# Baran-phys/IEA-GAN

Measured on AMD Instinct MI355X. Metric: events/sec (40x250x768) per G+D train step, higher is better.
Workload: dtype bf16; 1 GPU; BASELINE configs[1]: 1 event (40x1x256x768) per GPU per step, hinge loss only, RRM on, DiffAugment on, ortho reg + Adam + EMA in the timed region, fp32 master weights, 4 synthetic events in rotation; parallelism=dp1, hip_graph=True

## Files before the change

iea-gan_amd/_hip.py:

```python
from __future__ import annotations

import ctypes as C
import os

import torch

_HERE = os.path.dirname(os.path.abspath(__file__))
LIB_PATH = os.path.join(_HERE, "libieagan_hip.so")
CONV_FP8_NOSCALE = 8
CONV_FP8 = 4
CONV_FORCE_WS64 = 32
CONV_NO_WS64 = 16
CONV_NO_LDS_WEIGHTS = 2
CONV_FORCE_GATHER = 1
B1_TP32 = 4
BWD_NO_REDUCE = 16
PXD_BINS = 251
PXD_CLUSTER_COLUMNS = {"size_spectrum": (0, 64), "charge_spectrum": (64, 256), "seed_spectrum": (320, 256), "size_u_spectrum": (576, 32),
                       "size_v_spectrum": (608, 32)}
PXD_CLUSTER_BINS = 640
PXD_MAP_U, PXD_MAP_V = 25, 48
PXD_MATCH_COUNTERS = ("hits", "matched", "changed", "shared", "lost")
PXD_MATCH_COLUMNS = {"residual_u": (5, 64), "residual_v": (69, 64), "purity": (133, 32)}
PXD_MATCH_BINS = 165
PXD_CORR_MAX_COLUMNS, PXD_CORR_MAX_EVENTS = 1024, 65535
PROLOGUE_BWD_SLOTS = 64
AUG_SLOTS = 128
BNB_REPL = 8
STAT_REPL = 32
SN_FIELDS = 16

vp, fp, lp, ip = C.c_void_p, C.c_void_p, C.c_void_p, C.c_void_p


class SrcDesc(C.Structure):
    _fields_ = [("x", vp), ("Cx", C.c_int), ("Hs", C.c_int), ("Ws", C.c_int), ("rs", C.c_int),
                ("scale", vp), ("shift", vp), ("aff_nstride", C.c_int), ("relu", C.c_int)]


class ConvDesc(C.Structure):
    _fields_ = [("N", C.c_int), ("H", C.c_int), ("W", C.c_int), ("Cin", C.c_int), ("Cout", C.c_int),
                ("taps", C.c_int), ("Kpad", C.c_int), ("src", SrcDesc), ("w", vp), ("bias", vp),
                ("ra", vp), ("Cra", C.c_int), ("Ca", C.c_int), ("ra_rs", C.c_int), ("ra_scale", C.c_float), ("rb", vp),
                ("Crb", C.c_int), ("mask", vp), ("out", vp), ("stats", vp), ("n_per_event", C.c_int), ("flags", C.c_int),
                ("bnb_scale", vp), ("bnb_shift", vp), ("bnb_nstride", C.c_int), ("bnb_relu", C.c_int), ("stats_slots", C.c_int)]


class WgradDesc(C.Structure):
    _fields_ = [("N", C.c_int), ("H", C.c_int), ("W", C.c_int), ("Cin", C.c_int), ("Cout", C.c_int),
                ("taps", C.c_int), ("Kpad", C.c_int), ("src", SrcDesc), ("g", vp), ("Cg", C.c_int),
                ("dw", vp), ("tiles_per_block", C.c_int), ("pad_rows", C.c_int), ("partials", vp), ("colsum", vp)]


class Conv1x1BwdDesc(C.Structure):
    _fields_ = [("N", C.c_int), ("H", C.c_int), ("W", C.c_int), ("Cin", C.c_int), ("Cout", C.c_int), ("Kpad", C.c_int),
                ("Kpad2", C.c_int), ("src", SrcDesc), ("g", vp), ("Cg", C.c_int), ("y", vp), ("dstat", vp), ("n_per_event", C.c_int),
                ("geff_out", vp), ("w_bwd", vp), ("lg", vp), ("lC", C.c_int), ("lCa", C.c_int), ("lmode", C.c_int), ("dx", vp),
                ("out_mode", C.c_int), ("bn_acc", vp), ("dw", vp), ("partials", vp), ("colsum", vp), ("flags", C.c_int), ("bn_slots", C.c_int)]


class Conv3x3BwdDesc(C.Structure):
    _fields_ = [("N", C.c_int), ("H", C.c_int), ("W", C.c_int), ("C", C.c_int), ("Kpad", C.c_int), ("src", SrcDesc), ("g", vp), ("Cg", C.c_int),
                ("y", vp), ("dstat", vp), ("n_per_event", C.c_int), ("w_bwd", vp), ("dx", vp), ("bn_acc", vp), ("dw", vp), ("partials", vp),
                ("colsum", vp), ("flags", C.c_int), ("bn_slots", C.c_int)]


class ReduceItem(C.Structure):
    _fields_ = [("partials", vp), ("dw", vp), ("S", C.c_int), ("Cout", C.c_int), ("Kpad", C.c_int), ("K", C.c_int)]


class DStemDesc(C.Structure):
    _fields_ = [("img", vp), ("N", C.c_int), ("H", C.c_int), ("W", C.c_int), ("w_in", vp), ("b_in", vp), ("w1", vp), ("b1", vp), ("wsc", vp),
                ("bsc", vp), ("h1", vp), ("p0", vp), ("sc", vp), ("dh1", vp), ("dp0", vp), ("w1_bwd", vp), ("dw_in", vp), ("db_in", vp),
                ("dw1", vp), ("db1", vp)]


class ProfRec(C.Structure):
    _fields_ = [("name", C.c_char * 96), ("launches", C.c_long), ("ms", C.c_double),
                ("flops", C.c_double), ("bytes", C.c_double), ("bytes_min", C.c_double)]


ABI_VERSION = 12
i, f, l = C.c_int, C.c_float, C.c_long
_SIGS = {
    "ieagan_abi_version": [],
    "ieagan_prof_enable": [i],
    "ieagan_prof_reset": [],
    "ieagan_prof_collect": [C.POINTER(ProfRec), i],
    "ieagan_conv_forward": [C.POINTER(ConvDesc), vp],
    "ieagan_conv_wgrad": [C.POINTER(WgradDesc), i, vp],
    "ieagan_conv_wgrad_workspace": [C.POINTER(WgradDesc), i],
    "ieagan_conv1x1_bwd": [C.POINTER(Conv1x1BwdDesc), vp],
    "ieagan_conv1x1_bwd_workspace": [C.POINTER(Conv1x1BwdDesc)],
    "ieagan_conv1x1_bwd_supported": [i, i, i, i],
    "ieagan_conv3x3_bwd": [C.POINTER(Conv3x3BwdDesc), vp],
# ... 147 lines not shown
```

iea-gan_amd/csrc/conv3x3_ws.hip:

```cpp
#include "common.h"
#include "conv_args.h"
#include "conv3x3_tile.h"

#define WS_H 8
#define WS_W 32

template <bool AFF, bool RELU, int RS, int CIN, bool BNB, bool MPF, int NCW, bool FULL>
__global__ __launch_bounds__((NCW + 4) * 64, (NCW == 4 ? 4 : 3)) void conv3x3_ws_kernel(ConvArgs a, int tiles_w, int tiles_h, int tpe, int tpb, int nblk, int bpe) {
    constexpr int NT = CIN / 16;
    constexpr int AW = WS_W + 2, AH = WS_H + 2;
    constexpr int PS = CIN * 2 + 16;
    constexpr int KP = ((9 * CIN + 31) / 32) * 32;
    constexpr int WSB = KP * 2 + 16;
    constexpr int CH = CIN / 8;
    constexpr int TOT = AH * AW * CH;
    constexpr int PF = (TOT + 255) / 256;
    constexpr int HALO_BYTES = AH * AW * PS;
    extern __shared__ __attribute__((aligned(16))) char smem_all[];
    constexpr int RPW = WS_H / NCW, MTW = 2 * RPW;
    __shared__ float red[NCW * NT * 16 * 2];
    __shared__ __attribute__((aligned(32))) float aff_all[4 * 64];
    char* wlds = smem_all;
    char* halo0 = smem_all + NT * 16 * WSB;
    float* epi_all = (float*)(halo0 + 2 * HALO_BYTES);

    const int lane = threadIdx.x & 63, wave = threadIdx.x >> 6;
    const bool consumer = wave < NCW;
    const int lr = lane & 15, lg = lane >> 4;
    const int H = a.H, W = a.W;
    const TileRun run = tile_run(nblk, 1, bpe, tpe, tpb);
    const int t0 = run.t0, ntl = run.t1 - run.t0;

    for (int idx = threadIdx.x; idx < NT * 16 * (KP / 8); idx += (NCW + 4) * 64) {
        const int row = idx / (KP / 8), kc = idx - row * (KP / 8);
        *(bf16x8*)(wlds + row * WSB + kc * 16) = *(const bf16x8*)((const bf16*)a.w + (long)row * KP + kc * 8);
    }

    auto tile_coords = [&](int t, int& n, int& h0, int& w0) { tile_origin<WS_H, WS_W>(t, tiles_w, tiles_h, n, h0, w0); };

    if (!consumer) {
        const int ptid = threadIdx.x - NCW * 64;
        bf16x8 rawA[PF], rawB[PF];
        unsigned okA = 0, okB = 0;
        float* aff_w = aff_all + (wave & 3) * 64;
        int aff_n = -1;
        auto load_tile = [&](int t, bf16x8(&raw)[PF], unsigned& okmask) {
            int n, h0, w0;
            tile_coords(t, n, h0, w0);
            halo_request<RS, CH, AW, TOT, 256>(a.src, H, W, n, h0, w0, ptid, raw, okmask);
        };
        auto store_tile = [&](int t, const bf16x8(&raw)[PF], unsigned okmask, char* dst) {
            int n, h0, w0;
            tile_coords(t, n, h0, w0);
            if (AFF && n != aff_n) {
                wave_fence();
                const int c = lane & 31;
                if (c < CIN) aff_w[lane] = (lane < 32 ? a.src.scale : a.src.shift)[(long)n * a.src.aff_nstride + c];
                wave_fence();
                aff_n = n;
            }
#pragma unroll
            for (int j = 0; j < PF; ++j) {
                const int idx = ptid + j * 256;
                if (idx >= TOT) continue;
                const int hp = idx / CH, cc = idx - hp * CH;
                *(bf16x8*)(dst + hp * PS + cc * 16) = prologue_chunk<AFF, RELU>(raw[j], okmask & (1u << j), aff_w + cc * 8, aff_w + 32 + cc * 8);
            }
        };
        auto produce = [&](int r, bf16x8(&raw)[PF], unsigned& okmask) {
            if (r + 1 < ntl) store_tile(t0 + r + 1, raw, okmask, halo0 + ((r + 1) & 1) * HALO_BYTES);
            load_tile(t0 + min(r + 3, ntl - 1), raw, okmask);
        };
        if (ntl <= 0) {
            __syncthreads();
            return;
        }
        load_tile(t0, rawA, okA);
        store_tile(t0, rawA, okA, halo0);
        load_tile(t0 + min(1, ntl - 1), rawB, okB);
        load_tile(t0 + min(2, ntl - 1), rawA, okA);
        __syncthreads();
        for (int r = 0; r < ntl; r += 2) {
            produce(r, rawB, okB);
            __syncthreads();
            if (r + 1 >= ntl) break;
            produce(r + 1, rawA, okA);
            __syncthreads();
        }
        if (a.stats != nullptr) __syncthreads();
        return;
    }

    float s1[8], s2[8];
#pragma unroll
    for (int i = 0; i < 8; ++i) s1[i] = s2[i] = 0.f;
    int pbase[MTW];
#pragma unroll
    for (int mt = 0; mt < MTW; ++mt) pbase[mt] = ((RPW * wave + (mt >> 1)) * AW + (mt & 1) * 16 + lr) * PS;
    float* epi = epi_all + wave * EpiLds<NT>::FLOATS;
    constexpr int CPP = NT * 2, EIT = (32 * CPP) / 64;
    const int ecc = lane % CPP;
    float bias_r[8];
    load_bias8<NT>(a, 0, bias_r);
    constexpr bool has_mask = MPF;
    bf16x8 mk_cur[RPW * EIT], mk_nxt[RPW * EIT];
    auto mask_request = [&](int t, bf16x8(&mk)[RPW * EIT]) {
        int n, h0, w0;
        tile_coords(t, n, h0, w0);
#pragma unroll
        for (int half = 0; half < RPW; ++half)
#pragma unroll
            for (int it = 0; it < EIT; ++it) {
                const int hh = h0 + RPW * wave + half, ww = w0 + (it * 64 + lane) / CPP;
                if (FULL) {
                    mk[half * EIT + it] = *(const bf16x8*)((const bf16*)a.mask + (((long)n * H + hh) * W + ww) * CIN + ecc * 8);
                } else {
                    mk[half * EIT + it] = zero8();
                    if (hh < H && ww < W) mk[half * EIT + it] = *(const bf16x8*)((const bf16*)a.mask + (((long)n * H + hh) * W + ww) * CIN + ecc * 8);
                }
            }
    };
    if (has_mask && ntl > 0) mask_request(t0, mk_cur);
    __syncthreads();
    for (int r = 0; r < ntl; ++r) {
        const char* smem = halo0 + (r & 1) * HALO_BYTES;
        int n, h0, w0;
        tile_coords(t0 + r, n, h0, w0);
        f32x4 acc[MTW][NT];
#pragma unroll
        for (int mt = 0; mt < MTW; ++mt)
#pragma unroll
            for (int nt = 0; nt < NT; ++nt) acc[mt][nt] = (f32x4){0.f, 0.f, 0.f, 0.f};
        constexpr int KS = KP / 32;
        bf16x8 bq[CIN >= 32 ? 2 : 1][NT], aq[CIN >= 32 ? 2 : 1][MTW];
        auto ldb = [&](int ks, bf16x8(&b)[NT]) {
#pragma unroll
            for (int nt = 0; nt < NT; ++nt) b[nt] = *(const bf16x8*)(wlds + (nt * 16 + lr) * WSB + (ks * 32 + lg * 8) * 2);
        };
        auto lda = [&](int ks, bf16x8(&x)[MTW]) {
            const int k = ks * 32 + lg * 8;
            int tap = k / CIN;
            const int c = k - tap * CIN;
            const bool kval = tap < 9;
            if (!kval) tap = 0;
            const int toff = ((tap / 3) * AW + (tap - (tap / 3) * 3)) * PS + c * 2;
#pragma unroll
            for (int mt = 0; mt < MTW; ++mt) {
                x[mt] = *(const bf16x8*)(smem + pbase[mt] + toff);
                if (!kval) x[mt] = zero8();
            }
        };
        if constexpr (CIN >= 32) {
            ldb(0, bq[0]);
            lda(0, aq[0]);
#pragma unroll
            for (int ks = 0; ks < KS; ++ks) {
                if (ks + 1 < KS) {
                    ldb(ks + 1, bq[(ks + 1) & 1]);
                    lda(ks + 1, aq[(ks + 1) & 1]);
                }
                __builtin_amdgcn_sched_barrier(0);
#pragma unroll
                for (int mt = 0; mt < MTW; ++mt)
#pragma unroll
                    for (int nt = 0; nt < NT; ++nt)
                        acc[mt][nt] = __builtin_amdgcn_mfma_f32_16x16x32_bf16(aq[ks & 1][mt], bq[ks & 1][nt], acc[mt][nt], 0, 0, 0);
                __builtin_amdgcn_sched_barrier(0);
            }
        } else {
#pragma unroll
            for (int ks = 0; ks < KS; ++ks) {
                ldb(ks, bq[0]);
                lda(ks, aq[0]);
#pragma unroll
                for (int mt = 0; mt < MTW; ++mt)
#pragma unroll
                    for (int nt = 0; nt < NT; ++nt)
                        acc[mt][nt] = __builtin_amdgcn_mfma_f32_16x16x32_bf16(aq[0][mt], bq[0][nt], acc[mt][nt], 0, 0, 0);
            }
        }
#pragma unroll
        for (int half = 0; half < RPW; ++half) {
            const tile_pix<2, FULL> pix(n, h0, w0, 2 * (RPW * wave + half), H, W);
            const f32x4(&sub)[2][NT] = *reinterpret_cast<const f32x4(*)[2][NT]>(&acc[2 * half]);
            if (half == 0 && has_mask) mask_request(t0 + min(r + 1, ntl - 1), mk_nxt);
            if (has_mask) conv_epilogue<BNB, NT>(a, sub, epi, 0, pix, s1, s2, bias_r, &mk_cur[half * EIT]);
            else conv_epilogue<BNB, NT>(a, sub, epi, 0, pix, s1, s2, bias_r, nullptr);
        }
        if (has_mask) {
#pragma unroll
            for (int i = 0; i < RPW * EIT; ++i) mk_cur[i] = mk_nxt[i];
        }
        __syncthreads();
    }
    if (a.stats != nullptr && ntl > 0) stats_flush<NT, NCW>(a, s1, s2, 0, red, epi_all, run.bid, run.event);
}

template <bool AFF, bool RELU, int RS, bool BNB, bool MPF, bool FULL>
static int ws_launch_f(const ConvArgs& a, hipStream_t st) {
    const TilePlan p = tile_plan_events(a, WS_H, WS_W, a.Cin == 16 ? 512 : 256, 1);
#define WS_GO(CINV, NCWV)                                                                                                    \
    {                                                                                                                        \
        constexpr int NTV = CINV / 16;                                                                                       \
        constexpr int KPV = ((9 * CINV + 31) / 32) * 32;                                                                     \
        size_t tail = (size_t)NCWV * EpiLds<NTV>::FLOATS * 4;                                                                \
        if (tail < (size_t)NCWV * STATS_SX_FLOATS * 4) tail = (size_t)NCWV * STATS_SX_FLOATS * 4;                             \
        const size_t lds = (size_t)NTV * 16 * (KPV * 2 + 16) + 2 * (size_t)(WS_H + 2) * (WS_W + 2) * (CINV * 2 + 16) + tail;  \
        CONV_PLAN_POINT(p.bpe, 1)                                                                                            \
        constexpr auto kern = conv3x3_ws_kernel<AFF, RELU, RS, CINV, BNB, MPF, NCWV, FULL>;                                  \
        if (reserve_lds<kern>(lds, "conv3x3_ws") != 0) return IEAGAN_ELAUNCH;                                                \
        hipLaunchKernelGGL(kern, dim3(p.nblk), dim3((NCWV + 4) * 64), lds, st, a, p.tiles_w, p.tiles_h, p.tpe, p.tpb, p.nblk, p.bpe); \
    }
    WS_GO(16, 4)
#undef WS_GO
    return 1;
}

template <bool AFF, bool RELU, int RS, bool BNB, bool MPF>
static int ws_launch_c(const ConvArgs& a, hipStream_t st) {
    if (a.H % WS_H == 0 && a.W % WS_W == 0) return ws_launch_f<AFF, RELU, RS, BNB, MPF, true>(a, st);
    return ws_launch_f<AFF, RELU, RS, BNB, MPF, false>(a, st);
}

int conv3x3_ws_launch(const ConvArgs& a, hipStream_t st) {
    if (a.taps != 9 || a.Cin != a.Cout || a.Cin != 16 || a.src.rs == 2) return 0;
    if (a.Kpad != ((9 * a.Cin + 31) / 32) * 32 || a.src.Cx % 8 != 0) return 0;
    const int tiles = a.N * ((a.W + WS_W - 1) / WS_W) * ((a.H + WS_H - 1) / WS_H);
    if (tiles < 1024) return 0;
    const bool aff = a.src.scale != nullptr, relu = a.src.relu != 0;
    if (aff && !relu) return 0;
    if (a.mask != nullptr) {
        if (aff || relu || a.src.rs != 0) return 0;
        return a.bnb_scale != nullptr ? ws_launch_c<false, false, 0, true, true>(a, st) : ws_launch_c<false, false, 0, false, true>(a, st);
    }
    return dispatch_prologue(a, [&](auto AFF, auto RELU, auto RS, auto BNB) {
        if constexpr (BNB() || (AFF() && !RELU())) return 0;
        else return ws_launch_c<AFF(), RELU(), RS(), false, false>(a, st);
    });
}
```

iea-gan_amd/csrc/conv_igemm.hip:

```cpp
#include "common.h"
#include "conv_args.h"
#include "conv3x3_tile.h"
#include <stdio.h>

template <int TAPS, bool AFF, bool RELU, int RS, int NT, bool LAFF, bool BNB = false>
__global__ __launch_bounds__(256, 4) void conv_gather_kernel(ConvArgs a) {
    constexpr int EROWS = (NT >= 2) ? 16 : 32;
    __shared__ __attribute__((aligned(16))) float epi[4 * EROWS * EpiLds<NT>::LDW];
    __shared__ float red[4 * NT * 16 * 2];
    __shared__ __attribute__((aligned(32))) float aff_s[LAFF ? 2 * AFF_MAXC : 8];
    const int lane = threadIdx.x & 63, wave = threadIdx.x >> 6;
    const int lr = lane & 15, lg = lane >> 4;
    const int H = a.H, W = a.W, HW = H * W;
    const long M = (long)a.N * HW;
    const bool sk = NT == 1 && (a.flags & CONV_INTERNAL_SPLITK) != 0;
    const int ppb = sk ? 32 : 128;
    const long m_base = sk ? (long)blockIdx.x * 32 : ((long)blockIdx.x * 4 + wave) * 32;
    const int n_base = blockIdx.y * NT * 16;

    int pn[2], ph[2], pw[2];
    bool pv[2];
#pragma unroll
    for (int mt = 0; mt < 2; ++mt) {
        const long m = m_base + mt * 16 + lr;
// ... 299 lines not shown
                for (int nt = 0; nt < NT; ++nt) {
                    if (PF > 0) b[nt] = *(const bf16x8*)(smem_all + (nt * 16 + lr) * WS + (ks * 32 + lg * 8) * 2);
                    else b[nt] = *(const bf16x8*)(wnt[nt] + wlane + (unsigned)(ks * 64));
                }
            };
            auto lda = [&](int ks, bf16x8(&x)[4]) {
                const int tap = (ks * 32) / CIN, c0 = (ks * 32) % CIN;
                const int toff = ((tap / 3) * AW + (tap % 3)) * PSC + c0 * 2;
#pragma unroll
                for (int mt = 0; mt < 4; ++mt) x[mt] = *(const bf16x8*)(smem + pbase[mt] + lg * 16 + toff);
            };
            ldb(0, bq[0]);
            lda(0, aq[0]);
#pragma unroll
            for (int ks = 0; ks < KS; ++ks) {
                if (ks + 1 < KS) {
                    ldb(ks + 1, bq[(ks + 1) & 1]);
                    lda(ks + 1, aq[(ks + 1) & 1]);
                }
                __builtin_amdgcn_sched_barrier(0);
#pragma unroll
                for (int mt = 0; mt < 4; ++mt)
#pragma unroll
                    for (int nt = 0; nt < NT; ++nt)
                        acc[mt][nt] = __builtin_amdgcn_mfma_f32_16x16x32_bf16(aq[ks & 1][mt], bq[ks & 1][nt], acc[mt][nt], 0, 0, 0);
                __builtin_amdgcn_sched_barrier(0);
            }
        } else {
            for (int ks = 0; ks < ksteps; ++ks) kstep(ks);
        }
        __syncthreads();
        float* epi = (float*)smem + wave * EpiLds<NT>::FLOATS;
#pragma unroll
        for (int half = 0; half < 2; ++half) {
            const tile_pix<2, false> pix(n, h0, w0, 2 * (2 * wave + half), H, W);
            const f32x4(&sub)[2][NT] = *reinterpret_cast<const f32x4(*)[2][NT]>(&acc[2 * half]);
            conv_epilogue<BNB, NT, 2, false>(a, sub, epi, n_base, pix, s1, s2);
        }
        __syncthreads();
    }
    if (a.stats != nullptr && t0 < t1) stats_flush<NT>(a, s1, s2, n_base, red, (float*)smem, run.bid, run.event);
}

template <bool AFF, bool RELU, int RS, bool BNB = false>
static int launch_halo_nt(const ConvArgs& a, hipStream_t st) {
    const TilePlan g = tile_grid(a, HT_H, HT_W);
    const int ntiles = g.ntiles;
    const int tpb = ntiles / 2048 > 8 ? 8 : ntiles / 2048;
    const size_t halo = (size_t)(HT_H + 2) * (HT_W + 2) * (a.Cin * 2 + 16);
#define HALO_LAUNCH(NTV, PFV, CINV)                                                                              \
    {                                                                                                        \
        size_t lds = halo;                                                                                   \
        const size_t epi = (size_t)4 * EpiLds<NTV>::FLOATS * 4;                                              \
        if (epi > lds) lds = epi;                                                                            \
        if (lds < 4 * STATS_SX_FLOATS * 4) lds = 4 * STATS_SX_FLOATS * 4;                                    \
        if ((PFV) > 0) lds += (size_t)NTV * 16 * (a.Kpad * 2 + 16);                                          \
        const TilePlan p = tile_split(g, (PFV) > 0 ? tpb : 1);                                               \
        CONV_PLAN_POINT(p.bpe, 0)                                                                            \
        hipLaunchKernelGGL((conv3x3_halo_kernel<AFF, RELU, RS, NTV, PFV, CINV, BNB>), dim3(p.nblk, (a.Cout + 16 * NTV - 1) / (16 * NTV)), \
                           dim3(256), lds, st, a, p.tiles_w, p.tiles_h, p.tpe, p.tpb, p.nblk, p.bpe);        \
    }
    const bool small = ntiles * ((a.Cout + 63) / 64) < 512;
    const bool kp_ok = a.Kpad == ((9 * a.Cin + 31) / 32) * 32;
    if (!kp_ok) {
        if (a.Cout % 64 == 0 && !small) HALO_LAUNCH(4, 0, 0)
        else if (a.Cout % 32 == 0 && !(small && ntiles * (a.Cout / 32) < 512)) HALO_LAUNCH(2, 0, 0)
        else HALO_LAUNCH(1, 0, 0)
    }
    else if (a.Cin == 16 && a.Cout == 16) HALO_LAUNCH(1, 3, 16)
    else if (a.Cin == 32 && a.Cout == 32) HALO_LAUNCH(2, 6, 32)
    else if (a.Cin == 64 && a.Cout % 64 == 0 && !small) HALO_LAUNCH(4, 0, 64)
    else if (a.Cin == 128 && a.Cout % 64 == 0 && !small) HALO_LAUNCH(4, 0, 128)
    else if (a.Cin == 128 && a.Cout % 32 == 0 && !(small && ntiles * (a.Cout / 32) < 512)) HALO_LAUNCH(2, 0, 128)
    else if (a.Cin == 64 && a.Cout % 32 == 0 && !(small && ntiles * (a.Cout / 32) < 512)) HALO_LAUNCH(2, 0, 64)
    else if (a.Cout % 64 == 0 && !small) HALO_LAUNCH(4, 0, 0)
    else if (a.Cout % 32 == 0 && !(small && ntiles * (a.Cout / 32) < 512)) HALO_LAUNCH(2, 0, 0)
    else HALO_LAUNCH(1, 0, 0)
#undef HALO_LAUNCH
    return 0;
}

int conv_gather_launch(const ConvArgs& a, hipStream_t st) {
    CHECK_ARG(a.taps == 1 || a.taps == 9, "conv: taps must be 1 or 9 (got %d)", a.taps);
    CHECK_ARG((a.flags & ~(IEAGAN_CONV_FORCE_GATHER | IEAGAN_CONV_NO_LDS_WEIGHTS | IEAGAN_CONV_FP8 | IEAGAN_CONV_FP8_NOSCALE | IEAGAN_CONV_NO_WS64 | IEAGAN_CONV_FORCE_WS64)) == 0, "conv: unknown flag bits 0x%x", a.flags);
    CHECK_ARG(a.Cin % 8 == 0 && a.Cout % 8 == 0, "conv: Cin/Cout must be multiples of 8 (%d,%d)", a.Cin, a.Cout);
    CHECK_ARG(a.Kpad % 32 == 0 && a.Kpad >= a.taps * a.Cin, "conv: bad Kpad %d", a.Kpad);
    CHECK_ARG(a.src.rs >= 0 && a.src.rs <= 2, "conv: bad resample mode %d", a.src.rs);
    CHECK_ARG(a.src.Cx % 8 == 0, "conv: source channel stride must be a multiple of 8");
    CHECK_ARG((a.src.scale == nullptr) == (a.src.shift == nullptr), "conv: scale/shift must come together");
    if (a.src.rs == 1) CHECK_ARG(a.H == 2 * a.src.Hs && a.W == 2 * a.src.Ws, "conv: upsample geometry mismatch");
    if (a.src.rs == 2) CHECK_ARG(2 * a.H == a.src.Hs && 2 * a.W == a.src.Ws, "conv: pool geometry mismatch");
    if (a.src.rs == 0) CHECK_ARG(a.H == a.src.Hs && a.W == a.src.Ws, "conv: geometry mismatch");
    if (a.ra) CHECK_ARG(a.Ca <= a.Cout && a.Ca <= a.Cra && a.Ca % 8 == 0 && a.Cra % 8 == 0, "conv: residual channel slice out of range");
    if (a.ra && a.ra_rs == 1) CHECK_ARG(a.H % 2 == 0 && a.W % 2 == 0, "conv: upsampled residual needs even H, W");
    if (a.rb) CHECK_ARG(a.Crb % 8 == 0 && a.Crb >= a.Cout - a.Ca, "conv: bad residual-B channel count");
    CHECK_ARG(a.n_per_event >= 0 && (a.n_per_event == 0 || a.N % a.n_per_event == 0), "conv: N=%d is not a whole number of events of %d images", a.N, a.n_per_event);
    if (a.bnb_scale != nullptr)
        CHECK_ARG(a.src.scale == nullptr && a.src.relu == 0 && a.src.rs == 0 && a.bnb_shift != nullptr && a.mask != nullptr && a.stats != nullptr && a.n_per_event == 1 && a.bias == nullptr && a.Cout % 8 == 0 &&
                  (a.bnb_nstride == 0 || a.bnb_nstride >= a.Cout), "conv: BatchNorm-backward epilogue needs a plain prologue, shift, x (mask), per-image accumulators (n_per_event = 1), no bias");
    if (a.stats != nullptr && a.n_per_event > 0 && a.n_per_event < a.N)
        CHECK_ARG(((long)a.n_per_event * a.H * a.W) % 128 == 0, "conv: per-event statistics need n_per_event*H*W %% 128 == 0 (%d*%d*%d)", a.n_per_event, a.H, a.W);
    const double flops = 2.0 * a.N * a.H * a.W * (double)a.Cout * a.taps * a.Cin;
    double bytes = 2.0 * a.N * ((double)a.src.Hs * a.src.Ws * a.Cin + (double)a.H * a.W * a.Cout);
    const double bytes_min = bytes;
    if (a.mask) bytes += 2.0 * a.N * (double)a.H * a.W * a.Cout;
    if (a.ra) bytes += 2.0 * a.N * (double)a.H * a.W * a.Ca * (a.ra_rs == 1 ? 0.25 : (a.ra_rs == 2 ? 4.0 : 1.0));
    if (a.rb) bytes += 2.0 * a.N * (double)a.H * a.W * (a.Cout - a.Ca);
    const bool halo = a.taps == 9 && a.src.rs != 2 && a.W >= 16 && a.H >= 4 && a.Cin % 16 == 0 && !(a.flags & IEAGAN_CONV_FORCE_GATHER) &&
                      (size_t)(HT_H + 2) * (HT_W + 2) * (a.Cin * 2 + 16) <= 150 * 1024 && a.Cin <= AFF_MAXC;
    char tag[64] = "";
    if (prof_tags_on())
        snprintf(tag, sizeof(tag), "ci%d co%d %dx%d rs%d a%d r%d res%d%s", a.Cin, a.Cout, a.H, a.W, a.src.rs, a.src.scale != nullptr,
                 a.src.relu, a.ra ? a.ra_rs + 1 : 0, a.mask ? " mask" : "");
    ProfScope prof(a.taps == 9 ? (halo ? "conv3x3_halo" : "conv3x3_gather") : "conv1x1_gather", flops, bytes, st, tag, bytes_min);
    int rc;
    if (halo) {
        rc = (a.flags & IEAGAN_CONV_NO_LDS_WEIGHTS) ? 0 : conv3x3_ws64_launch(a, st);
        if (rc < 0) return rc;
        if (rc == 0) rc = (a.flags & IEAGAN_CONV_NO_LDS_WEIGHTS) ? 0 : conv3x3_lds_launch(a, st);
        if (rc < 0) return rc;
        if (rc == 0 && !(a.flags & IEAGAN_CONV_NO_LDS_WEIGHTS)) rc = conv3x3_ws_launch(a, st);
        if (rc < 0) return rc;
        if (rc == 0) rc = dispatch_prologue(a, [&](auto AFF, auto RELU, auto RS, auto BNB) { return launch_halo_nt<AFF(), RELU(), RS(), BNB()>(a, st); });
        else rc = 0;
    } else if (a.taps == 9) {
        if (a.src.rs == 0) rc = launch_gather_pro<9, 0>(a, st);
        else if (a.src.rs == 1) rc = launch_gather_pro<9, 1>(a, st);
        else { ieagan_set_error("conv: 3x3 with pooled source is not instantiated"); return IEAGAN_EINVAL; }
    } else {
        if (a.src.rs == 0) {
            if (!(a.flags & IEAGAN_CONV_FORCE_GATHER) && conv1x1_stream_launch(a, st)) rc = 0;
            else if (!(a.flags & IEAGAN_CONV_FORCE_GATHER) && conv1x1_tile_launch(a, st)) rc = 0;
            else rc = launch_gather_pro<1, 0>(a, st);
        }
        else if (a.src.rs == 2) {
            if (!(a.flags & IEAGAN_CONV_FORCE_GATHER) && conv1x1_tile_launch(a, st)) rc = 0;
            else rc = launch_gather_pro<1, 2>(a, st);
        }
        else { ieagan_set_error("conv: 1x1 with upsampled source is not instantiated"); return IEAGAN_EINVAL; }
    }
    if (conv_plan_ctx().on) return rc;
    CHECK_LAUNCH("conv_forward");
    return rc;
}
```

include/ieagan_hip.h:

```cpp
#ifndef IEAGAN_HIP_H
#define IEAGAN_HIP_H
#include <stddef.h>
#ifdef __cplusplus
extern "C" {
#endif

const char* ieagan_last_error(void);
#define IEAGAN_ABI_VERSION 12
int ieagan_abi_version(void);

int ieagan_prof_enable(int on);
int ieagan_prof_reset(void);
typedef struct { char name[96]; long launches; double ms; double flops; double bytes; double bytes_min; } ieagan_prof_rec;
int ieagan_prof_collect(ieagan_prof_rec* out, int cap);

typedef struct {
    const void* x;
    int Cx, Hs, Ws;
    int rs;
    const float* scale;
    const float* shift;
    int aff_nstride;
    int relu;
} ieagan_src_desc;

typedef struct {
    int N, H, W;
    int Cin, Cout, taps;
    int Kpad;
    ieagan_src_desc src;
    const void* w;
    const float* bias;
    const void* ra;
    int Cra, Ca, ra_rs;
    float ra_scale;
    const void* rb;
    int Crb;
    const void* mask;
    void* out;
    float* stats;
    int n_per_event;
    int flags;
    const float* bnb_scale;
    const float* bnb_shift;
    int bnb_nstride;
    int bnb_relu;
    int stats_slots;
} ieagan_conv_desc;
#define IEAGAN_CONV_FORCE_GATHER 1
#define IEAGAN_CONV_FP8 4
#define IEAGAN_CONV_FP8_NOSCALE 8
#define IEAGAN_CONV_NO_LDS_WEIGHTS 2
#define IEAGAN_CONV_NO_WS64 16
#define IEAGAN_CONV_FORCE_WS64 32
int ieagan_conv_forward(const ieagan_conv_desc* d, void* stream);
int ieagan_conv_stats_slots(const ieagan_conv_desc* d);

typedef struct {
    int N, H, W;
    int Cin, Cout, taps, Kpad;
    ieagan_src_desc src;
    const void* g;
    int Cg;
    float* dw;
    int tiles_per_block;
    int pad_rows;
    float* partials;
    float* colsum;
} ieagan_wgrad_desc;
int ieagan_conv_wgrad(const ieagan_wgrad_desc* d, int use_tr_read, void* stream);
long ieagan_conv_wgrad_workspace(const ieagan_wgrad_desc* d, int use_tr_read);

typedef struct {
    int N, H, W;
    int Cin, Cout, Kpad, Kpad2;
    ieagan_src_desc src;
    const void* g;
    int Cg;
    const void* y;
    const float* dstat;
    int n_per_event;
    void* geff_out;
    const void* w_bwd;
    const void* lg;
    int lC, lCa, lmode;
    void* dx;
    int out_mode;
    float* bn_acc;
    float* dw;
    float* partials;
    float* colsum;
    int flags;
    int bn_slots;
} ieagan_conv1x1_bwd_desc;
#define IEAGAN_B1_TP32 4
#define IEAGAN_BWD_NO_REDUCE 16
int ieagan_conv1x1_bwd(const ieagan_conv1x1_bwd_desc* d, void* stream);
long ieagan_conv1x1_bwd_workspace(const ieagan_conv1x1_bwd_desc* d);
int ieagan_conv1x1_bwd_supported(int Cin, int Cout, int rs, int affine);
int ieagan_conv1x1_bwd_slots(const ieagan_conv1x1_bwd_desc* d);
int ieagan_wgrad_reduce(const float* partials, float* dw, int S, int Cout, int Kpad, int K, void* stream);
typedef struct {
    const float* partials;
    float* dw;
    int S, Cout, Kpad, K;
} ieagan_reduce_item;
int ieagan_wgrad_reduce_batched(const ieagan_reduce_item* items, int n, void* stream);

typedef struct {
    int N, H, W;
    int C, Kpad;
    ieagan_src_desc src;
    const void* g;
    int Cg;
    const void* y;
    const float* dstat;
    int n_per_event;
    const void* w_bwd;
    void* dx;
    float* bn_acc;
    float* dw;
    float* partials;
    float* colsum;
    int flags;
    int bn_slots;
} ieagan_conv3x3_bwd_desc;
int ieagan_conv3x3_bwd(const ieagan_conv3x3_bwd_desc* d, void* stream);
long ieagan_conv3x3_bwd_workspace(const ieagan_conv3x3_bwd_desc* d);
int ieagan_conv3x3_bwd_supported(int C, int rs, int affine, int relu, int effgrad, int H, int W);
int ieagan_conv3x3_bwd_slots(const ieagan_conv3x3_bwd_desc* d);

int ieagan_effgrad(const void* dout, const void* out, const float* dstat, void* geff, float* colsum,
                   long P, int C, int E, void* stream);
#define IEAGAN_PROLOGUE_BWD_SLOTS 64
int ieagan_prologue_bwd(const void* da, const void* x, int Cx, const float* scale, const float* shift,
                        int nstride, int relu, int rs, void* dx, float* dscale, float* dshift,
                        int N, int Hs, int Ws, int C, const void* radd, int Cr, int Ca, int rmode, int slots, void* stream);
// ... 184 lines not shown
```

Measured before the change: 31.66 events/s.

## Move conv3x3 warp-specialized epilogue onto mover waves to overlap with MFMA

In the warp-specialized 16-channel 3x3 conv, when there is no residual, the consumer waves now write their raw accumulators to LDS. The producer (mover) waves then run the bias, BatchNorm-backward, mask and statistics epilogue for the previous tile while consumers start the next tile's MFMA loop. This takes epilogue work off the MFMA waves, at the cost of a second block barrier per tile and more LDS for the per-wave epilogue buffers. A static_assert checks that both roles hit the same number of barriers. The change also adds FORCE_WS and NO_WS flags and templates the tile shape.

```diff
diff --git a/iea-gan_amd/_hip.py b/iea-gan_amd/_hip.py
--- a/iea-gan_amd/_hip.py
+++ b/iea-gan_amd/_hip.py
@@ -11,6 +11,8 @@
 CONV_FP8 = 4
 CONV_FORCE_WS64 = 32
 CONV_NO_WS64 = 16
+CONV_FORCE_WS = 64
+CONV_NO_WS = 128
 CONV_NO_LDS_WEIGHTS = 2
 CONV_FORCE_GATHER = 1
 B1_TP32 = 4
diff --git a/iea-gan_amd/csrc/conv3x3_ws.hip b/iea-gan_amd/csrc/conv3x3_ws.hip
--- a/iea-gan_amd/csrc/conv3x3_ws.hip
+++ b/iea-gan_amd/csrc/conv3x3_ws.hip
@@ -5,10 +5,49 @@
 #define WS_H 8
 #define WS_W 32
 
-template <bool AFF, bool RELU, int RS, int CIN, bool BNB, bool MPF, int NCW, bool FULL>
+constexpr int ws_barriers_mover(int ntl, bool stats, bool ho) {
+    if (ntl <= 0) return 0;
+    int n = 1;
+    if (ho) {
+        n += 2;
+        for (int r = 1; r < ntl; r += 2) {
+            n += 2;
+            if (r + 1 >= ntl) break;
+            n += 2;
+        }
+    } else {
+        for (int r = 0; r < ntl; r += 2) {
+            n += 1;
+            if (r + 1 >= ntl) break;
+            n += 1;
+        }
+    }
+    if (stats) n += 1;
+    return n;
+}
+constexpr int ws_barriers_consumer(int ntl, bool stats, bool ho) {
+    if (ntl <= 0) return 0;
+    int n = 1;
+    for (int r = 0; r < ntl; ++r) n += ho ? 2 : 1;
+    if (stats) n += 1;
+    return n;
+}
+constexpr bool ws_barriers_agree() {
+    for (int ntl = 0; ntl <= 9; ++ntl)
+        for (int s = 0; s < 2; ++s)
+            for (int ho = 0; ho < 2; ++ho)
+                if (ws_barriers_mover(ntl, s != 0, ho != 0) != ws_barriers_consumer(ntl, s != 0, ho != 0)) return false;
+    return true;
+}
+static_assert(ws_barriers_agree(), "conv3x3_ws: movers and consumers must execute the same number of block barriers");
+
+template <bool AFF, bool RELU, int RS, int CIN, bool BNB, bool MPF, int NCW, bool FULL, int TH, int TW, bool HO>
 __global__ __launch_bounds__((NCW + 4) * 64, (NCW == 4 ? 4 : 3)) void conv3x3_ws_kernel(ConvArgs a, int tiles_w, int tiles_h, int tpe, int tpb, int nblk, int bpe) {
+    static_assert(TW == 16 || TW == 32, "one or two m-tiles per tile row");
+    static_assert(TH % NCW == 0 && (TH / NCW) * (TW / 16) % 2 == 0, "a consumer wave owns whole pairs of m-tiles");
+    static_assert(!HO || NCW == 4, "mover wave 4 + w finishes the buffers of consumer wave w");
     constexpr int NT = CIN / 16;
-    constexpr int AW = WS_W + 2, AH = WS_H + 2;
+    constexpr int AW = TW + 2, AH = TH + 2;
     constexpr int PS = CIN * 2 + 16;
     constexpr int KP = ((9 * CIN + 31) / 32) * 32;
     constexpr int WSB = KP * 2 + 16;
@@ -17,7 +56,9 @@
     constexpr int PF = (TOT + 255) / 256;
     constexpr int HALO_BYTES = AH * AW * PS;
     extern __shared__ __attribute__((aligned(16))) char smem_all[];
-    constexpr int RPW = WS_H / NCW, MTW = 2 * RPW;
+    constexpr int RPW = TH / NCW, MPR = TW / 16;
+    constexpr int MTW = RPW * MPR, EH = MTW / 2;
+    constexpr int EPW = (HO ? EH : 1) * EpiLds<NT>::FLOATS;
     __shared__ float red[NCW * NT * 16 * 2];
     __shared__ __attribute__((aligned(32))) float aff_all[4 * 64];
     char* wlds = smem_all;
@@ -30,13 +71,34 @@
     const int H = a.H, W = a.W;
     const TileRun run = tile_run(nblk, 1, bpe, tpe, tpb);
     const int t0 = run.t0, ntl = run.t1 - run.t0;
+    if (ntl <= 0) return;
 
     for (int idx = threadIdx.x; idx < NT * 16 * (KP / 8); idx += (NCW + 4) * 64) {
         const int row = idx / (KP / 8), kc = idx - row * (KP / 8);
         *(bf16x8*)(wlds + row * WSB + kc * 16) = *(const bf16x8*)((const bf16*)a.w + (long)row * KP + kc * 8);
     }
 
-    auto tile_coords = [&](int t, int& n, int& h0, int& w0) { tile_origin<WS_H, WS_W>(t, tiles_w, tiles_h, n, h0, w0); };
+    auto tile_coords = [&](int t, int& n, int& h0, int& w0) { tile_origin<TH, TW>(t, tiles_w, tiles_h, n, h0, w0); };
+
+    constexpr int CPP = NT * 2, EIT = (32 * CPP) / 64;
+    const int ecc = lane % CPP;
+    auto mask_request = [&](int t, int cw, bf16x8(&mk)[EH * EIT]) __attribute__((always_inline)) {
+        int n, h0, w0;
+        tile_coords(t, n, h0, w0);
+#pragma unroll
+        for (int e = 0; e < EH; ++e)
+#pragma unroll
+            for (int it = 0; it < EIT; ++it) {
+                const int row = (it * 64 + lane) / CPP;
+                const int hh = h0 + (MPR == 2 ? RPW * cw + e : RPW * cw + 2 * e + (row >> 4)), ww = w0 + (MPR == 2 ? row : (row & 15));
+                if (FULL) {
+                    mk[e * EIT + it] = *(const bf16x8*)((const bf16*)a.mask + (((long)n * H + hh) * W + ww) * CIN + ecc * 8);
+                } else {
+                    mk[e * EIT + it] = zero8();
+                    if (hh < H && ww < W) mk[e * EIT + it] = *(const bf16x8*)((const bf16*)a.mask + (((long)n * H + hh) * W + ww) * CIN + ecc * 8);
+                }
+            }
+    };
 
     if (!consumer) {
         const int ptid = threadIdx.x - NCW * 64;
@@ -44,12 +106,12 @@
         unsigned okA = 0, okB = 0;
         float* aff_w = aff_all + (wave & 3) * 64;
         int aff_n = -1;
-        auto load_tile = [&](int t, bf16x8(&raw)[PF], unsigned& okmask) {
+        auto load_tile = [&](int t, bf16x8(&raw)[PF], unsigned& okmask) __attribute__((always_inline)) {
             int n, h0, w0;
             tile_coords(t, n, h0, w0);
             halo_request<RS, CH, AW, TOT, 256>(a.src, H, W, n, h0, w0, ptid, raw, okmask);
         };
-        auto store_tile = [&](int t, const bf16x8(&raw)[PF], unsigned okmask, char* dst) {
+        auto store_tile = [&](int t, const bf16x8(&raw)[PF], unsigned okmask, char* dst) __attribute__((always_inline)) {
             int n, h0, w0;
             tile_coords(t, n, h0, w0);
             if (AFF && n != aff_n) {
@@ -67,66 +129,85 @@
                 *(bf16x8*)(dst + hp * PS + cc * 16) = prologue_chunk<AFF, RELU>(raw[j], okmask & (1u << j), aff_w + cc * 8, aff_w + 32 + cc * 8);
             }
         };
-        auto produce = [&](int r, bf16x8(&raw)[PF], unsigned& okmask) {
-            if (r + 1 < ntl) store_tile(t0 + r + 1, raw, okmask, halo0 + ((r + 1) & 1) * HALO_BYTES);
-            load_tile(t0 + min(r + 3, ntl - 1), raw, okmask);
-        };
-        if (ntl <= 0) {
-            __syncthreads();
-            return;
-        }
         load_tile(t0, rawA, okA);
         store_tile(t0, rawA, okA, halo0);
         load_tile(t0 + min(1, ntl - 1), rawB, okB);
         load_tile(t0 + min(2, ntl - 1), rawA, okA);
-        __syncthreads();
-        for (int r = 0; r < ntl; r += 2) {
-            produce(r, rawB, okB);
-            __syncthreads();
-            if (r + 1 >= ntl) break;
-            produce(r + 1, rawA, okA);
-            __syncthreads();
-        }
-        if (a.stats != nullptr) __syncthreads();
+        if constexpr (HO) {
+            const int wl = wave - NCW;
+            float* epi = epi_all + wl * EPW;
+            float s1[8], s2[8];
+#pragma unroll
+            for (int i = 0; i < 8; ++i) s1[i] = s2[i] = 0.f;
+            bf16x8 mk[EH * EIT];
+            int bnb_n = -1;
+            ConvArgs ae = a;
+            ae.ra = nullptr;
+            ae.rb = nullptr;
+            if (!MPF) ae.mask = nullptr;
+            if (BNB) ae.bias = nullptr;
+            float bias_r[8];
+            load_bias8<NT>(ae, 0, bias_r);
+            auto finish = [&](int t) __attribute__((always_inline)) {
+                int n, h0, w0;
+                tile_coords(t, n, h0, w0);
+                if (BNB && n != bnb_n) {
+                    wave_fence();
+                    if (lane < 2 * CIN) aff_w[lane] = (lane < CIN ? a.bnb_scale : a.bnb_shift)[(long)n * a.bnb_nstride + (lane < CIN ? lane : lane - CIN)];
+                    wave_fence();
+                    bnb_n = n;
+                }
+#pragma unroll
+                for (int e = 0; e < EH; ++e) {
+                    const tile_pix<MPR, FULL> pix(n, h0, w0, MTW * wl + 2 * e, H, W);
+                    if constexpr (BNB) conv_epilogue_finish<true, NT>(ae, epi + e * EpiLds<NT>::FLOATS, 0, pix, s1, s2, bias_r, &mk[e * EIT], aff_w);
+                    else if constexpr (MPF) conv_epilogue_finish<false, NT>(ae, epi + e * EpiLds<NT>::FLOATS, 0, pix, s1, s2, bias_r, &mk[e * EIT]);
+                    else conv_epilogue_finish<false, NT>(ae, epi + e * EpiLds<NT>::FLOATS, 0, pix, s1, s2, bias_r, nullptr);
+                }
+            };
+            auto step = [&](int r, bf16x8(&raw)[PF], unsigned& okmask) __attribute__((always_inline)) {
+                if (r + 1 < ntl) store_tile(t0 + r + 1, raw, okmask, halo0 + ((r + 1) & 1) * HALO_BYTES);
+                load_tile(t0 + min(r + 3, ntl - 1), raw, okmask);
+                if (r > 0) finish(t0 + r - 1);
+                if (MPF) mask_request(t0 + r, wl, mk);
+                __syncthreads();
+                __syncthreads();
+            };
+            __syncthreads();
+            step(0, rawB, okB);
+            for (int r = 1; r < ntl; r += 2) {
+                step(r, rawA, okA);
+                if (r + 1 >= ntl) break;
+                step(r + 1, rawB, okB);
+            }
+            finish(t0 + ntl - 1);
+            if (a.stats != nullptr) {
+                stats_fold<NT>(s1, s2, red, epi, wl);
+                __syncthreads();
+            }
+        } else {
+            auto produce = [&](int r, bf16x8(&raw)[PF], unsigned& okmask) __attribute__((always_inline)) {
+                if (r + 1 < ntl) store_tile(t0 + r + 1, raw, okmask, halo0 + ((r + 1) & 1) * HALO_BYTES);
+                load_tile(t0 + min(r + 3, ntl - 1), raw, okmask);
+            };
+            __syncthreads();
+            for (int r = 0; r < ntl; r += 2) {
+                produce(r, rawB, okB);
+                __syncthreads();
+                if (r + 1 >= ntl) break;
+                produce(r + 1, rawA, okA);
+                __syncthreads();
+            }
+            if (a.stats != nullptr) __syncthreads();
+        }
         return;
     }
 
-    float s1[8], s2[8];
-#pragma unroll
-    for (int i = 0; i < 8; ++i) s1[i] = s2[i] = 0.f;
     int pbase[MTW];
 #pragma unroll
-    for (int mt = 0; mt < MTW; ++mt) pbase[mt] = ((RPW * wave + (mt >> 1)) * AW + (mt & 1) * 16 + lr) * PS;
-    float* epi = epi_all + wave * EpiLds<NT>::FLOATS;
-    constexpr int CPP = NT * 2, EIT = (32 * CPP) / 64;
-    const int ecc = lane % CPP;
-    float bias_r[8];
-    load_bias8<NT>(a, 0, bias_r);
-    constexpr bool has_mask = MPF;
-    bf16x8 mk_cur[RPW * EIT], mk_nxt[RPW * EIT];
-    auto mask_request = [&](int t, bf16x8(&mk)[RPW * EIT]) {
-        int n, h0, w0;
-        tile_coords(t, n, h0, w0);
-#pragma unroll
-        for (int half = 0; half < RPW; ++half)
-#pragma unroll
-            for (int it = 0; it < EIT; ++it) {
-                const int hh = h0 + RPW * wave + half, ww = w0 + (it * 64 + lane) / CPP;
-                if (FULL) {
-                    mk[half * EIT + it] = *(const bf16x8*)((const bf16*)a.mask + (((long)n * H + hh) * W + ww) * CIN + ecc * 8);
-                } else {
-                    mk[half * EIT + it] = zero8();
-                    if (hh < H && ww < W) mk[half * EIT + it] = *(const bf16x8*)((const bf16*)a.mask + (((long)n * H + hh) * W + ww) * CIN + ecc * 8);
-                }
-            }
-    };
-    if (has_mask && ntl > 0) mask_request(t0, mk_cur);
-    __syncthreads();
-    for (int r = 0; r < ntl; ++r) {
-        const char* smem = halo0 + (r & 1) * HALO_BYTES;
-        int n, h0, w0;
-        tile_coords(t0 + r, n, h0, w0);
-        f32x4 acc[MTW][NT];
+    for (int mt = 0; mt < MTW; ++mt) pbase[mt] = ((RPW * wave + mt / MPR) * AW + (mt % MPR) * 16 + lr) * PS;
+    float* epi = epi_all + wave * EPW;
+    auto kloop = [&](const char* smem, f32x4(&acc)[MTW][NT]) __attribute__((always_inline)) {
 #pragma unroll
         for (int mt = 0; mt < MTW; ++mt)
 #pragma unroll
@@ -179,54 +260,92 @@
                         acc[mt][nt] = __builtin_amdgcn_mfma_f32_16x16x32_bf16(aq[0][mt], bq[0][nt], acc[mt][nt], 0, 0, 0);
             }
         }
-#pragma unroll
-        for (int half = 0; half < RPW; ++half) {
-            const tile_pix<2, FULL> pix(n, h0, w0, 2 * (RPW * wave + half), H, W);
-            const f32x4(&sub)[2][NT] = *reinterpret_cast<const f32x4(*)[2][NT]>(&acc[2 * half]);
-            if (half == 0 && has_mask) mask_request(t0 + min(r + 1, ntl - 1), mk_nxt);
-            if (has_mask) conv_epilogue<BNB, NT>(a, sub, epi, 0, pix, s1, s2, bias_r, &mk_cur[half * EIT]);
-            else conv_epilogue<BNB, NT>(a, sub, epi, 0, pix, s1, s2, bias_r, nullptr);
-        }
-        if (has_mask) {
-#pragma unroll
-            for (int i = 0; i < RPW * EIT; ++i) mk_cur[i] = mk_nxt[i];
-        }
+    };
+
+    if constexpr (HO) {
         __syncthreads();
-    }
-    if (a.stats != nullptr && ntl > 0) stats_flush<NT, NCW>(a, s1, s2, 0, red, epi_all, run.bid, run.event);
-}
-
-template <bool AFF, bool RELU, int RS, bool BNB, bool MPF, bool FULL>
+        for (int r = 0; r < ntl; ++r) {
+            f32x4 acc[MTW][NT];
+            kloop(halo0 + (r & 1) * HALO_BYTES, acc);
+            __syncthreads();
+#pragma unroll
+            for (int e = 0; e < EH; ++e)
+                conv_epilogue_put<NT>(*reinterpret_cast<const f32x4(*)[2][NT]>(&acc[2 * e]), epi + e * EpiLds<NT>::FLOATS);
+            __syncthreads();
+        }
+        if (a.stats != nullptr) {
+            __syncthreads();
+            stats_add<NT, NCW>(a, 0, red, run.bid, run.event);
+        }
+    } else {
+        float s1[8], s2[8];
+#pragma unroll
+        for (int i = 0; i < 8; ++i) s1[i] = s2[i] = 0.f;
+        float bias_r[8];
+        load_bias8<NT>(a, 0, bias_r);
+        bf16x8 mk_cur[EH * EIT], mk_nxt[EH * EIT];
+        if (MPF) mask_request(t0, wave, mk_cur);
+        __syncthreads();
+        for (int r = 0; r < ntl; ++r) {
+            int n, h0, w0;
+            tile_coords(t0 + r, n, h0, w0);
+            f32x4 acc[MTW][NT];
+            kloop(halo0 + (r & 1) * HALO_BYTES, acc);
+#pragma unroll
+            for (int e = 0; e < EH; ++e) {
+                const tile_pix<MPR, FULL> pix(n, h0, w0, MTW * wave + 2 * e, H, W);
+                const f32x4(&sub)[2][NT] = *reinterpret_cast<const f32x4(*)[2][NT]>(&acc[2 * e]);
+                if (e == 0 && MPF) mask_request(t0 + min(r + 1, ntl - 1), wave, mk_nxt);
+                if (MPF) conv_epilogue<BNB, NT>(a, sub, epi, 0, pix, s1, s2, bias_r, &mk_cur[e * EIT]);
+                else conv_epilogue<BNB, NT>(a, sub, epi, 0, pix, s1, s2, bias_r, nullptr);
+            }
+            if (MPF) {
+#pragma unroll
+                for (int i = 0; i < EH * EIT; ++i) mk_cur[i] = mk_nxt[i];
+            }
+            __syncthreads();
+        }
+        if (a.stats != nullptr) stats_flush<NT, NCW>(a, s1, s2, 0, red, epi_all, run.bid, run.event);
+    }
+}
+
+template <int CIN, int NCW, int TH, int TW, bool HO>
+constexpr size_t ws_lds_bytes() {
+    constexpr int NT = CIN / 16, KP = ((9 * CIN + 31) / 32) * 32;
+    constexpr size_t epi = (size_t)NCW * (HO ? (TH / NCW) * (TW / 16) / 2 : 1) * EpiLds<NT>::FLOATS * 4, fold = (size_t)NCW * STATS_SX_FLOATS * 4;
+    return (size_t)NT * 16 * (KP * 2 + 16) + 2 * (size_t)(TH + 2) * (TW + 2) * (CIN * 2 + 16) + (epi > fold ? epi : fold);
+}
+static_assert(2 * (ws_lds_bytes<16, 4, WS_H, WS_W, true>() + 2 * 1024) <= 160 * 1024, "conv3x3_ws: two blocks must share a CU");
+static_assert(EpiLds<1>::FLOATS * (WS_H / 4) * (WS_W / 16) / 2 >= STATS_SX_FLOATS, "a mover folds its statistics in the transpose buffers it has read");
+
+template <bool AFF, bool RELU, int RS, bool BNB, bool MPF, bool FULL, bool HO>
 static int ws_launch_f(const ConvArgs& a, hipStream_t st) {
-    const TilePlan p = tile_plan_events(a, WS_H, WS_W, a.Cin == 16 ? 512 : 256, 1);
-#define WS_GO(CINV, NCWV)                                                                                                    \
-    {                                                                                                                        \
-        constexpr int NTV = CINV / 16;                                                                                       \
-        constexpr int KPV = ((9 * CINV + 31) / 32) * 32;                                                                     \
-        size_t tail = (size_t)NCWV * EpiLds<NTV>::FLOATS * 4;                                                                \
-        if (tail < (size_t)NCWV * STATS_SX_FLOATS * 4) tail = (size_t)NCWV * STATS_SX_FLOATS * 4;                             \
-        const size_t lds = (size_t)NTV * 16 * (KPV * 2 + 16) + 2 * (size_t)(WS_H + 2) * (WS_W + 2) * (CINV * 2 + 16) + tail;  \
-        CONV_PLAN_POINT(p.bpe, 1)                                                                                            \
-        constexpr auto kern = conv3x3_ws_kernel<AFF, RELU, RS, CINV, BNB, MPF, NCWV, FULL>;                                  \
-        if (reserve_lds<kern>(lds, "conv3x3_ws") != 0) return IEAGAN_ELAUNCH;                                                \
-        hipLaunchKernelGGL(kern, dim3(p.nblk), dim3((NCWV + 4) * 64), lds, st, a, p.tiles_w, p.tiles_h, p.tpe, p.tpb, p.nblk, p.bpe); \
-    }
-    WS_GO(16, 4)
-#undef WS_GO
+    const TilePlan p = tile_plan_events(a, WS_H, WS_W, 512, (a.flags & IEAGAN_CONV_FORCE_WS) ? 4 : 1);
+    constexpr size_t lds = ws_lds_bytes<16, 4, WS_H, WS_W, HO>();
+    CONV_PLAN_POINT(p.bpe, 1)
+    constexpr auto kern = conv3x3_ws_kernel<AFF, RELU, RS, 16, BNB, MPF, 4, FULL, WS_H, WS_W, HO>;
+    if (reserve_lds<kern>(lds, "conv3x3_ws") != 0) return IEAGAN_ELAUNCH;
+    hipLaunchKernelGGL(kern, dim3(p.nblk), dim3(512), lds, st, a, p.tiles_w, p.tiles_h, p.tpe, p.tpb, p.nblk, p.bpe);
     return 1;
 }
 
 template <bool AFF, bool RELU, int RS, bool BNB, bool MPF>
 static int ws_launch_c(const ConvArgs& a, hipStream_t st) {
-    if (a.H % WS_H == 0 && a.W % WS_W == 0) return ws_launch_f<AFF, RELU, RS, BNB, MPF, true>(a, st);
-    return ws_launch_f<AFF, RELU, RS, BNB, MPF, false>(a, st);
+    const bool full = a.H % WS_H == 0 && a.W % WS_W == 0;
+    if constexpr (!AFF) {
+        if (a.ra == nullptr && a.rb == nullptr)
+            return full ? ws_launch_f<AFF, RELU, RS, BNB, MPF, true, true>(a, st) : ws_launch_f<AFF, RELU, RS, BNB, MPF, false, true>(a, st);
+    }
+    if constexpr (BNB || MPF) return 0;
+    else return full ? ws_launch_f<AFF, RELU, RS, BNB, MPF, true, false>(a, st) : ws_launch_f<AFF, RELU, RS, BNB, MPF, false, false>(a, st);
 }
 
 int conv3x3_ws_launch(const ConvArgs& a, hipStream_t st) {
+    if (a.flags & IEAGAN_CONV_NO_WS) return 0;
     if (a.taps != 9 || a.Cin != a.Cout || a.Cin != 16 || a.src.rs == 2) return 0;
     if (a.Kpad != ((9 * a.Cin + 31) / 32) * 32 || a.src.Cx % 8 != 0) return 0;
     const int tiles = a.N * ((a.W + WS_W - 1) / WS_W) * ((a.H + WS_H - 1) / WS_H);
-    if (tiles < 1024) return 0;
+    if (tiles < 1024 && !(a.flags & IEAGAN_CONV_FORCE_WS)) return 0;
     const bool aff = a.src.scale != nullptr, relu = a.src.relu != 0;
     if (aff && !relu) return 0;
     if (a.mask != nullptr) {
diff --git a/iea-gan_amd/csrc/conv_igemm.hip b/iea-gan_amd/csrc/conv_igemm.hip
--- a/iea-gan_amd/csrc/conv_igemm.hip
+++ b/iea-gan_amd/csrc/conv_igemm.hip
@@ -405,7 +405,7 @@
 
 int conv_gather_launch(const ConvArgs& a, hipStream_t st) {
     CHECK_ARG(a.taps == 1 || a.taps == 9, "conv: taps must be 1 or 9 (got %d)", a.taps);
-    CHECK_ARG((a.flags & ~(IEAGAN_CONV_FORCE_GATHER | IEAGAN_CONV_NO_LDS_WEIGHTS | IEAGAN_CONV_FP8 | IEAGAN_CONV_FP8_NOSCALE | IEAGAN_CONV_NO_WS64 | IEAGAN_CONV_FORCE_WS64)) == 0, "conv: unknown flag bits 0x%x", a.flags);
+    CHECK_ARG((a.flags & ~(IEAGAN_CONV_FORCE_GATHER | IEAGAN_CONV_NO_LDS_WEIGHTS | IEAGAN_CONV_FP8 | IEAGAN_CONV_FP8_NOSCALE | IEAGAN_CONV_NO_WS64 | IEAGAN_CONV_FORCE_WS64 | IEAGAN_CONV_NO_WS | IEAGAN_CONV_FORCE_WS)) == 0, "conv: unknown flag bits 0x%x", a.flags);
     CHECK_ARG(a.Cin % 8 == 0 && a.Cout % 8 == 0, "conv: Cin/Cout must be multiples of 8 (%d,%d)", a.Cin, a.Cout);
     CHECK_ARG(a.Kpad % 32 == 0 && a.Kpad >= a.taps * a.Cin, "conv: bad Kpad %d", a.Kpad);
     CHECK_ARG(a.src.rs >= 0 && a.src.rs <= 2, "conv: bad resample mode %d", a.src.rs);
diff --git a/include/ieagan_hip.h b/include/ieagan_hip.h
--- a/include/ieagan_hip.h
+++ b/include/ieagan_hip.h
@@ -53,6 +53,8 @@
 #define IEAGAN_CONV_NO_LDS_WEIGHTS 2
 #define IEAGAN_CONV_NO_WS64 16
 #define IEAGAN_CONV_FORCE_WS64 32
+#define IEAGAN_CONV_NO_WS 128
+#define IEAGAN_CONV_FORCE_WS 64
 int ieagan_conv_forward(const ieagan_conv_desc* d, void* stream);
 int ieagan_conv_stats_slots(const ieagan_conv_desc* d);
 
```

Result: no change. 31.83 events/s, median of 6 (+0.5%).
